# stm233/image-compression-for-machine

Measured on AMD Instinct MI355X. Metric: images/sec (256x256) cnn-hyperprior (WACNN) training step, higher is better.
Workload: dtype f32; 1 GPU; cnn (WACNN N=192 M=320) train step, lambda=0.0067 MSE, batch 16/GPU synthetic 256x256, Adam lr 1e-4 + aux Adam, clip 1.0; global_batch=16, parallelism=dp1

## Files before the change

### image-compression-for-machine_amd/csrc/conv_igemm.hip

```cpp
#include <cstdlib>
#include <vector>
#include "conv_common.h"

namespace icm {

template <int WCO, int WPX, int TCO, int TPX, int KS = 1>
__global__ __launch_bounds__(512, (TCO * TPX <= 3) ? 4 : 2) void conv_igemm_kernel(const ConvDesc d) {
  extern __shared__ __attribute__((aligned(16))) float smem[];
  static_assert(WCO * WPX * KS == 4, "4 MFMA waves per workgroup");
  constexpr int BCO_T = WCO * TCO;
  constexpr int TS = (TCO * TPX == 1) ? 3 : ((TCO * TPX == 2) ? 2 : 1);
  const int tid = threadIdx.x, lane = tid & 63, wave = tid >> 6;
  const bool loader = wave >= 4;
  const ConvPtrs P = d.g[blockIdx.y];
  const PatchGeom& pg = d.pg;

  int bid = xcd_block_id();
  const int cb = bid % d.ncb;
  int pt = bid / d.ncb;
  const int tx_i = pt % d.tiles_x;
  pt /= d.tiles_x;
  const int ty_i = pt % d.tiles_y;
  const int tn_i = pt / d.tiles_y;
  const int ox0 = tx_i << d.lgTW, oy0 = ty_i << d.lgTH, n0 = tn_i << d.lgTI;
  const int S_in = pg.S == 2 ? 2 : 1;
  const int iyb = oy0 * S_in + d.iy0, ixb = ox0 * S_in + d.ix0;
  const int bufsz = d.ckm * 8 * pg.CS;
  const int nchunks = (d.nchunks8 + d.ckm - 1) / d.ckm;

  if (loader) {
    const int lw = __builtin_amdgcn_readfirstlane(wave) - 4;
    PlaneMap pm;

    if (pg.dma) {
      plane_map_init(pm, pg, n0, iyb, ixb, lane);
      stage_planes_dma(P.x, pm, pg, 0, min(d.ckm, d.nchunks8) * 8, smem, lw, lane);
      asm volatile("s_waitcnt vmcnt(0)" ::: "memory");
      __syncthreads();
      for (int chunk = 0; chunk < nchunks; ++chunk) {
        if (chunk + 1 < nchunks) {
          const int c8 = (chunk + 1) * d.ckm;
          stage_planes_dma(P.x, pm, pg, c8 * 8, min(d.ckm, d.nchunks8 - c8) * 8, smem + ((chunk + 1) & 1) * bufsz, lw, lane);
          asm volatile("s_waitcnt vmcnt(0)" ::: "memory");
        }
        __syncthreads();
      }
      return;
    }
    if (pg.vec4) {
      plane_map_init_v4(pm, pg, n0, iyb, ixb, lane);
      stage_planes_v4<8>(P.x, pm, pg, 0, min(d.ckm, d.nchunks8) * 8, smem, lw);
      __syncthreads();
      for (int chunk = 0; chunk < nchunks; ++chunk) {
        if (chunk + 1 < nchunks) {
          const int c8 = (chunk + 1) * d.ckm;
          stage_planes_v4<8>(P.x, pm, pg, c8 * 8, min(d.ckm, d.nchunks8 - c8) * 8, smem + ((chunk + 1) & 1) * bufsz,
                             lw);
        }
        __syncthreads();
      }
      return;
    }
    plane_map_init(pm, pg, n0, iyb, ixb, lane);
    stage_planes<12>(P.x, pm, pg, 0, min(d.ckm, d.nchunks8) * 8, smem, lw);
    __syncthreads();
    for (int chunk = 0; chunk < nchunks; ++chunk) {
      if (chunk + 1 < nchunks) {
        const int c8 = (chunk + 1) * d.ckm;
        stage_planes<12>(P.x, pm, pg, c8 * 8, min(d.ckm, d.nchunks8 - c8) * 8, smem + ((chunk + 1) & 1) * bufsz, lw);
      }
      __syncthreads();
    }
    return;
  }

  const int wave_u = __builtin_amdgcn_readfirstlane(wave);
  const int wk = wave_u % KS, wsp = wave_u / KS;
  const int wco = wsp / WPX, wpx = wsp % WPX;
  const int h = lane >> 5, l31 = lane & 31;
  const int TWm = (1 << d.lgTW) - 1, THm = (1 << d.lgTH) - 1;
  const int rowmul = S_in * pg.PWrow;
  int boff[TPX];
#pragma unroll
  for (int tp = 0; tp < TPX; ++tp) {
    const int p = (wpx * TPX + tp) * 32 + l31;
    const int tx = p & TWm, ty = (p >> d.lgTW) & THm, ti = p >> (d.lgTW + d.lgTH);
    boff[tp] = h * pg.CS + ti * pg.PP + ty * rowmul + tx;
  }
  f32x16 acc[TCO][TPX];
#pragma unroll
  for (int a = 0; a < TCO; ++a)
#pragma unroll
    for (int b = 0; b < TPX; ++b)
#pragma unroll
      for (int r = 0; r < 16; ++r) acc[a][b][r] = 0.0f;

  const char* wbase = reinterpret_cast<const char*>(P.wp);
  const int cot0 = cb * BCO_T + wco * TCO;
  unsigned wl[TCO];
#pragma unroll
  for (int a = 0; a < TCO; ++a) wl[a] = (unsigned)(min(cot0 + a, d.ncot - 1) * 64 + lane) * 16u;
  const long long qstride = (long long)d.ncot * 64 * 16;
  const int Qtot = d.nchunks8 * d.ntaps;
  {
    int step_lane;
    {
      const int sq = lane / d.ntaps, tq = lane - sq * d.ntaps;
      step_lane = sq * 8 * pg.CS + d.tapoff[tq];
    }
    auto chunk_nq = [&](int c) { return min(d.ckm, d.nchunks8 - c * d.ckm) * d.ntaps; };
    auto steps2 = [&](int nq_c) { return ((((nq_c - wk + KS - 1) / KS) + TS - 1) / TS + 1) & ~1; };
    auto wptr = [&](int c, int st, int u) -> const char* {
      int nq_c = chunk_nq(c);
      const int ns2 = steps2(nq_c);
      if (st >= ns2) {
        st -= ns2;
        c += 1;
        nq_c = (c < nchunks) ? chunk_nq(c) : 1;
      }
      const int qw = min(c * d.ckm * d.ntaps + min((st * TS + u) * KS + wk, nq_c - 1), Qtot - 1);
      return wbase + qw * qstride;
    };
    f32x4 aq0[TS][TCO], aq1[TS][TCO];
#pragma unroll
    for (int u = 0; u < TS; ++u)
#pragma unroll
      for (int a = 0; a < TCO; ++a) {
        aq0[u][a] = *reinterpret_cast<const f32x4*>(wptr(0, 0, u) + wl[a]);
        aq1[u][a] = *reinterpret_cast<const f32x4*>(wptr(0, 1, u) + wl[a]);
      }

    __syncthreads();
    for (int chunk = 0; chunk < nchunks; ++chunk) {
      const float* cur = smem + (chunk & 1) * bufsz;
      const int nq = chunk_nq(chunk);
      const int nsteps2 = steps2(nq);
      float bv_n[TS][4][TPX];
      float ok_n[TS];
      auto bload = [&](int st, int u) {
        const int qq = (st * TS + u) * KS + wk;
        const int qc = min(qq, nq - 1);
        ok_n[u] = (qq < nq) ? 1.0f : 0.0f;
        const float* bp = cur + __builtin_amdgcn_readlane(step_lane, qc);
#pragma unroll
        for (int j = 0; j < 4; ++j)
#pragma unroll
          for (int tp = 0; tp < TPX; ++tp) bv_n[u][j][tp] = bp[boff[tp] + 2 * j * pg.CS];
      };
      auto half_step = [&](f32x4 (&aq)[TS][TCO], int st) {
        float bv[TS][4][TPX];
#pragma unroll
        for (int u = 0; u < TS; ++u)
#pragma unroll
          for (int j = 0; j < 4; ++j)
#pragma unroll
            for (int tp = 0; tp < TPX; ++tp) bv[u][j][tp] = bv_n[u][j][tp] * ok_n[u];
        const int stn = min(st + 1, nsteps2 - 1);
#pragma unroll
        for (int u = 0; u < TS; ++u) {
          const char* sp = wptr(chunk, st + 2, u);
#pragma unroll
          for (int a = 0; a < TCO; ++a) {
#pragma unroll
            for (int tp = 0; tp < TPX; ++tp)
#pragma unroll
              for (int j = 0; j < 4; ++j)
                acc[a][tp] = __builtin_amdgcn_mfma_f32_32x32x2f32(aq[u][a][j], bv[u][j][tp], acc[a][tp], 0, 0, 0);
            if (a == 0) bload(stn, u);
            aq[u][a] = *reinterpret_cast<const f32x4*>(sp + wl[a]);
            __builtin_amdgcn_sched_barrier(0);
          }
        }
      };
#pragma unroll
      for (int u = 0; u < TS; ++u) bload(0, u);
      for (int st = 0; st < nsteps2; st += 2) {
        half_step(aq0, st);
        half_step(aq1, st + 1);
      }
      __syncthreads();
    }
  }

  if constexpr (KS > 1) {
    static_assert(TCO == 1 && TPX == 1, "split-K configurations hold one tile per wave");
    float* red = smem + (wsp * (KS - 1)) * 1024;
    if (wk > 0) {
#pragma unroll
      for (int r = 0; r < 16; ++r) red[(wk - 1) * 1024 + r * 64 + lane] = acc[0][0][r];
    }
    __syncthreads();
    if (wk > 0) return;
#pragma unroll
    for (int k = 0; k < KS - 1; ++k)
#pragma unroll
      for (int r = 0; r < 16; ++r) acc[0][0][r] += red[k * 1024 + r * 64 + lane];
  }
  {
    int pn[TPX], poy[TPX], pox[TPX];
    bool pv[TPX];
#pragma unroll
    for (int tp = 0; tp < TPX; ++tp) {
      const int p = (wpx * TPX + tp) * 32 + l31;
      const int tx = p & TWm, ty = (p >> d.lgTW) & THm, ti = p >> (d.lgTW + d.lgTH);
      const int oyv = oy0 + ty, oxv = ox0 + tx;
      pn[tp] = n0 + ti;
      pv[tp] = (pn[tp] < d.pg.N) && (oyv < d.OHv) && (oxv < d.OWv);
      poy[tp] = oyv * d.out_sy + d.out_oy;
      pox[tp] = oxv * d.out_sx + d.out_ox;
    }
    epilogue_dispatch<TCO, TPX>(d, P, acc, cot0, h, pn, poy, pox, pv);
  }
}

struct PackDesc {
  const float* w;
  float* wp;
  int Co, Ci, KHW, src_out_major, ntaps, ncot, nchunks, nonneg;
  float bound, pedestal;
  int src_ld, src_off;
  int dst_ncot, dst_cot_off;
  int wino;
  short tapidx[ICM_MAX_TAPS];
};

#define ICM_PACK_LDS (8 * 32 * ICM_MAX_TAPS + 64)
__device__ __forceinline__ void pack_unit(const PackDesc& d, int cot, int chunk, float* lds) {
  const int KHW = d.KHW, tid = threadIdx.x;
  const int co0 = cot * 32, ci0 = chunk * 8;
  int rows, rlen, rstride;
  if (d.src_out_major) { rows = 32; rlen = 8 * KHW; } else { rows = 8; rlen = 32 * KHW; }
  rstride = rlen | 1;
  const int total = rows * rlen;
  for (int e0 = tid; e0 < total; e0 += 8 * (int)blockDim.x) {
    float v[8];
    int lo[8];
#pragma unroll
    for (int u = 0; u < 8; ++u) {
      const int e = e0 + u * (int)blockDim.x;
      v[u] = 0.0f;
      lo[u] = -1;
      if (e < total) {
        const int r = e / rlen, c = e - r * rlen;
        lo[u] = r * rstride + c;
        if (d.src_out_major) {
          const int co = co0 + r, ci = ci0 + c / KHW;
          if (co < d.Co && ci < d.Ci) v[u] = d.w[((long long)co * d.src_ld + d.src_off + ci0) * KHW + c];
        } else {
          const int ci = ci0 + r, co = co0 + c / KHW;
          if (ci < d.Ci && co < d.Co) v[u] = d.w[((long long)ci * d.src_ld + d.src_off + co0) * KHW + c];
        }
      }
    }
#pragma unroll
    for (int u = 0; u < 8; ++u) {
      if (lo[u] >= 0) {
        float x = v[u];
        if (d.nonneg) {
          x = fmaxf(x, d.bound);
          x = x * x - d.pedestal;
        }
        lds[lo[u]] = x;
      }
    }
  }
  __syncthreads();
  f32x4* out = reinterpret_cast<f32x4*>(d.wp);
  for (int e = tid; e < d.ntaps * 64; e += blockDim.x) {
    const int t = e >> 6, lane = e & 63;
    const int col = lane & 31, hh = lane >> 5, k = d.tapidx[t];
    f32x4 o;
#pragma unroll
    for (int j = 0; j < 4; ++j) {
      const int cil = 2 * j + hh;
      const float* gsrc = d.src_out_major ? lds + col * rstride + cil * KHW : lds + cil * rstride + col * KHW;
      float v;
      if (d.wino) {
        const int wa = t >> 2, wb = t & 3;
        float row[3];
#pragma unroll
        for (int p = 0; p < 3; ++p) {
          const float g0 = gsrc[d.wino == 2 ? (2 - p) * 3 + 2 : p * 3 + 0];
          const float g1 = gsrc[d.wino == 2 ? (2 - p) * 3 + 1 : p * 3 + 1];
          const float g2 = gsrc[d.wino == 2 ? (2 - p) * 3 + 0 : p * 3 + 2];
          row[p] = wb == 0 ? g0 : (wb == 3 ? g2 : (wb == 1 ? 0.5f * ((g0 + g2) + g1) : 0.5f * ((g0 + g2) - g1)));
        }
        v = wa == 0 ? row[0] : (wa == 3 ? row[2] : (wa == 1 ? 0.5f * ((row[0] + row[2]) + row[1]) : 0.5f * ((row[0] + row[2]) - row[1])));
      } else {
        v = gsrc[k];
      }
      const bool valid = (co0 + col < d.Co) && (ci0 + cil < d.Ci);
      o[j] = valid ? v : 0.0f;
    }
    out[((long long)(chunk * d.ntaps + t) * d.dst_ncot + d.dst_cot_off + cot) * 64 + lane] = o;
  }
  __syncthreads();
}

__global__ __launch_bounds__(256) void pack_weights_kernel(const PackDesc d) {
  __shared__ float lds[ICM_PACK_LDS];
  const int units = d.ncot * d.nchunks;
  for (int u = blockIdx.x; u < units; u += gridDim.x) pack_unit(d, u % d.ncot, u / d.ncot, lds);
}

#define ICM_PACK_NB 24
struct PackMulti {
  PackDesc g[ICM_PACK_NB];
};
__global__ __launch_bounds__(256) void pack_weights_multi_kernel(const PackMulti m) {
  __shared__ float lds[ICM_PACK_LDS];
  const PackDesc& d = m.g[blockIdx.y];
  const int units = d.ncot * d.nchunks;
  for (int u = blockIdx.x; u < units; u += gridDim.x) pack_unit(d, u % d.ncot, u / d.ncot, lds);
}

struct Tap {
  int kidx;
  int dy, dx;
};
struct ConvClass {
  int cy, cx;
  int iy0, ix0;
  int ey, ex;
  std::vector<Tap> taps;
};

static void axis_taps(int K, int s, int pad, int c, std::vector<int>& ks, std::vector<int>& dis) {
  for (int k = 0; k < K; ++k) {
    const int v = c + pad - k;
    if (((v % s) + s) % s != 0) continue;
    ks.push_back(k);
    dis.push_back(v >= 0 ? v / s : -((-v) / s));
  }
}

static std::vector<ConvClass> build_classes(int KH, int KW, int stride, int pad, int transposed) {
  std::vector<ConvClass> out;
  if (!transposed) {
    ConvClass c;
    c.cy = c.cx = 0;
    c.iy0 = c.ix0 = -pad;
    c.ey = KH;
    c.ex = KW;
    for (int kh = 0; kh < KH; ++kh)
      for (int kw = 0; kw < KW; ++kw) c.taps.push_back({kh * KW + kw, kh, kw});
    out.push_back(c);
    return out;
  }
  for (int cy = 0; cy < stride; ++cy)
    for (int cx = 0; cx < stride; ++cx) {
      std::vector<int> khs, dys, kws, dxs;
      axis_taps(KH, stride, pad, cy, khs, dys);
      axis_taps(KW, stride, pad, cx, kws, dxs);
      ConvClass c;
      c.cy = cy;
      c.cx = cx;
      int miny = 0, minx = 0, maxy = 0, maxx = 0;
      for (size_t i = 0; i < dys.size(); ++i) {
        miny = i ? std::min(miny, dys[i]) : dys[i];
        maxy = i ? std::max(maxy, dys[i]) : dys[i];
      }
      for (size_t i = 0; i < dxs.size(); ++i) {
        minx = i ? std::min(minx, dxs[i]) : dxs[i];
        maxx = i ? std::max(maxx, dxs[i]) : dxs[i];
      }
      c.iy0 = miny;
      c.ix0 = minx;
      c.ey = maxy - miny + 1;
      c.ex = maxx - minx + 1;
      for (size_t a = 0; a < khs.size(); ++a)
        for (size_t b = 0; b < kws.size(); ++b)
          c.taps.push_back({khs[a] * KW + kws[b], dys[a] - miny, dxs[b] - minx});
      out.push_back(c);
    }
  return out;
}

struct KernelCfg {
  int wco, wpx, tco, tpx;
  void (*fn)(const ConvDesc);
  int ks;
  double eff;
  int occ;
};
static const KernelCfg kCfgs[] = {
    {1, 4, 3, 2, conv_igemm_kernel<1, 4, 3, 2>, 1, 0.75, 1},
    {1, 4, 6, 1, conv_igemm_kernel<1, 4, 6, 1>, 1, 1.00, 1},
    {1, 4, 2, 2, conv_igemm_kernel<1, 4, 2, 2>, 1, 0.80, 1},
    {1, 4, 1, 2, conv_igemm_kernel<1, 4, 1, 2>, 1, 0.60, 2},
    {1, 4, 3, 1, conv_igemm_kernel<1, 4, 3, 1>, 1, 1.10, 2},
    {1, 4, 5, 1, conv_igemm_kernel<1, 4, 5, 1>, 1, 0.65, 1},
    {2, 2, 2, 1, conv_igemm_kernel<2, 2, 2, 1>, 1, 0.80, 2},
    {2, 2, 1, 1, conv_igemm_kernel<2, 2, 1, 1>, 1, 0.80, 2},
    {4, 1, 1, 1, conv_igemm_kernel<4, 1, 1, 1>, 1, 0.75, 2},
    {1, 4, 1, 1, conv_igemm_kernel<1, 4, 1, 1>, 1, 0.70, 2},
    {2, 1, 1, 1, conv_igemm_kernel<2, 1, 1, 1, 2>, 2, 0.70, 2},
    {1, 2, 1, 1, conv_igemm_kernel<1, 2, 1, 1, 2>, 2, 0.70, 2},
    {1, 1, 1, 1, conv_igemm_kernel<1, 1, 1, 1, 4>, 4, 0.65, 2},
};
constexpr int kNumCfgs = (int)(sizeof(kCfgs) / sizeof(kCfgs[0]));
static_assert(kNumCfgs <= ICM_CONV_CFG_KS8_64X64, "the K-split ids lie above the table rows");

static int g_force_cfg = ICM_CONV_CFG_AUTO;
static bool cfg_forced() { return g_force_cfg != ICM_CONV_CFG_AUTO; }
static bool ks8_forced() { return g_force_cfg == ICM_CONV_CFG_KS8_64X64 || g_force_cfg == ICM_CONV_CFG_KS8_32X128; }
static bool row_forced() { return cfg_forced() && g_force_cfg < ICM_CONV_CFG_KS8_64X64; }
static int g_force_1x1 = env_int("ICM_CONV_1X1", -1);

static Geometry make_geometry(int bpx, int OHv, int OWv, int N, int S, int ey, int ex, int nchunks8, int ntaps,
                              int tiles_per_wave) {
  Geometry g;
  const int lgB = ceil_log2(bpx);
  g.lgTW = std::min(std::min(5, lgB), ceil_log2(OWv));
  g.lgTH = std::min(lgB - g.lgTW, ceil_log2(OHv));
  g.lgTI = lgB - g.lgTW - g.lgTH;
  const int TW = 1 << g.lgTW, TH = 1 << g.lgTH, TI = 1 << g.lgTI;
  g.PW = (TW - 1) * S + ex;
  g.PH = (TH - 1) * S + ey;
  g.PWh = (g.PW + 1) / 2;
  g.PWrow = (S == 2) ? 2 * g.PWh : g.PW;
  g.PP = g.PH * g.PWrow;
  g.CS = TI * g.PP;
  g.tiles_x = cdiv(OWv, TW);
  g.tiles_y = cdiv(OHv, TH);
  g.tiles_n = cdiv(N, TI);
  int ckm = cdiv(256, ntaps * 4 * tiles_per_wave);
  ckm = std::max(1, std::min(ckm, nchunks8));
  ckm = std::max(1, std::min(ckm, 64 / std::max(1, ntaps)));
  while (ckm > 1 && (size_t)2 * ckm * 8 * g.CS * sizeof(float) > 64 * 1024) --ckm;
  g.ckm = ckm;
  g.lds_bytes = (size_t)2 * ckm * 8 * g.CS * sizeof(float);
  return g;
}
static bool fits_plane_map(const Geometry& g) { return (1 << g.lgTI) * g.PH * g.PW <= ICM_MAXJ * 64; }
static bool linear_patch(const Geometry& g) { return g.PWrow == g.PW && g.PP == g.PH * g.PW; }
static long long tile_count(const Geometry& g) { return (long long)g.tiles_x * g.tiles_y * g.tiles_n; }

struct ClassShape { int OHv, OWv, ncot, nchunks8, ntaps; };
static ClassShape class_shape(const icm_conv_args& a, const ConvClass& cls, int out_s) {
  return {a.transposed ? cdiv(a.OH - cls.cy, out_s) : a.OH, a.transposed ? cdiv(a.OW - cls.cx, out_s) : a.OW,
          cdiv(a.Cout, 32), cdiv(a.Cin, 8), (int)cls.taps.size()};
}

static int search_staged(const icm_conv_args& a, int ngroups, const ConvClass& cls, const ClassShape& s, int S_in,
                         Geometry& bg) {
  static const double kCoResBoost = env_double("ICM_CONV_BOOST", 1.25);
  int best = -1, best1 = -1;
  double best_cost = 1e300, best1_cost = 1e300;
  Geometry bg1{};
  for (int i = 0; i < kNumCfgs; ++i) {
    if (row_forced() && i != g_force_cfg) continue;
    const KernelCfg& c = kCfgs[i];
    const int bpx = c.wpx * c.tpx * 32, bco_t = c.wco * c.tco;
    Geometry g = make_geometry(bpx, s.OHv, s.OWv, a.N, S_in, cls.ey, cls.ex, s.nchunks8, s.ntaps, c.tco * c.tpx);
    if (c.ks > 1) g.lds_bytes = std::max<size_t>(g.lds_bytes, (size_t)(c.ks - 1) * c.wco * c.wpx * 4096);
    if (g.lds_bytes > 160 * 1024 || !fits_plane_map(g)) continue;
    const long long blocks = cdiv(s.ncot, bco_t) * tile_count(g) * ngroups;
    const int occ_max = (g.lds_bytes * 2 <= 160 * 1024) ? c.occ : 1;
    const int occ = (int)std::min<long long>(occ_max, (blocks + 255) / 256);
    const double rounds = (double)((blocks + 256 * occ - 1) / (256 * occ));
    const double mfma = (double)c.tco * c.tpx * s.nchunks8 * s.ntaps * 4 / c.ks + (c.ks > 1 ? 24.0 : 0.0);
    const double boost = occ > 1 ? 1.0 + (kCoResBoost - 1.0) * std::min(1.0, 1500.0 / mfma) : 1.0;
    const double cost = rounds * (occ * mfma / (c.eff * boost) + 200.0);
    if (s.ntaps >= 9 && (long long)s.OHv * s.OWv * a.N >= 16384 && cdiv(s.ncot, bco_t) == 1 && cost < best1_cost) {
      best1_cost = cost;
      best1 = i;
      bg1 = g;
    }
    if (cost < best_cost) {
      best_cost = cost;
      best = i;
      bg = g;
    }
  }
  if (best1 >= 0 && best1_cost <= 1.2 * best_cost) {
    best = best1;
    bg = bg1;
  }
  return best;
}

static int plan_ks8(const icm_conv_args& a, int ngroups, const ConvClass& cls, const ClassShape& s, int S_in, Geometry& g) {
  static const int ks8_on = env_int("ICM_CONV_KS8", 1);
  static const long long ks8_max = env_ll("ICM_CONV_KS8_MAXWG", 256);
  static const long long ks8_min = env_ll("ICM_CONV_KS8_MINWG", 160);
  if (!(ks8_forced() || (ks8_on && !cfg_forced())) || S_in != 1 || s.ntaps <= 1 || a.pro_act != ICM_ACT_NONE ||
      !EpiKs8::has(a.epi) || a.x_seg_len != 0)
    return 0;
  const int tco = g_force_cfg == ICM_CONV_CFG_KS8_32X128 ? 1 : (g_force_cfg == ICM_CONV_CFG_KS8_64X64 ? 2 : (s.ncot >= 2 ? 2 : 1));
  g = make_geometry(tco == 2 ? 64 : 128, s.OHv, s.OWv, a.N, S_in, cls.ey, cls.ex, s.nchunks8, s.ntaps, 4);
  int ckm = std::max(1, std::min(s.nchunks8, 64 / s.ntaps));
  while (ckm > 1 && (size_t)2 * ckm * 8 * g.CS * sizeof(float) > 96 * 1024) --ckm;
  g.ckm = ckm;
  g.lds_bytes = std::max((size_t)2 * ckm * 8 * g.CS * sizeof(float), (size_t)8 * 4 * 16 * 64 * sizeof(float));
  const long long blocks = cdiv(s.ncot, tco) * tile_count(g) * ngroups;
  const bool fits = g.lds_bytes <= 160 * 1024 && fits_plane_map(g) && linear_patch(g);
  return (fits && (ks8_forced() || (blocks <= ks8_max && blocks >= ks8_min && tco == 2))) ? tco : 0;
}

static int plan_class(const icm_conv_args& a, int ngroups, const ConvClass& cls, int S_in, int out_s, bool x_aligned16,
                      ConvPlan& p) {
  p = ConvPlan{};
  const ClassShape s = class_shape(a, cls, out_s);
  if (s.OHv <= 0 || s.OWv <= 0) return ICM_OK;
  if (s.ntaps > ICM_MAX_TAPS) return ICM_ERR_UNSUPPORTED;
  if (s.ntaps == 1 && S_in == 1 && out_s == 1 && cls.iy0 == 0 && cls.ix0 == 0 && a.x_seg_len == 0 && !cfg_forced()) {
    const int rc = plan_conv1x1(a, ngroups, g_force_1x1, p);
    if (rc >= 0) return rc;
  }
  p.row = search_staged(a, ngroups, cls, s, S_in, p.g);
  if (p.row < 0) return ICM_ERR_UNSUPPORTED;
  p.block = 512;
  Geometry kg;
  if (const int tco = plan_ks8(a, ngroups, cls, s, S_in, kg)) {
    p.family = kFamKs8;
    p.row = tco;
    p.g = kg;
    p.dma = 1;
  } else {
    const Geometry& g = p.g;
    const int plane4 = (1 << g.lgTI) * g.PH * (g.PW / 4);
    p.vec4 = S_in == 1 && cls.ex == 1 && cls.ey == 1 && cls.ix0 == 0 && (g.PW % 4) == 0 && ((1 << g.lgTW) % 4) == 0 &&
             (a.W % 4) == 0 && (a.x_bs % 4) == 0 && ((long long)a.H * a.W % 4) == 0 && plane4 <= 4 * 64 &&
             (g.CS % 4) == 0 && (g.PWrow % 4) == 0 && (g.PP % 4) == 0 && x_aligned16 && a.x_seg_len == 0;
    static const int dma_on = env_int("ICM_CONV_DMA", 1);
    p.dma = dma_on && !p.vec4 && S_in == 1 && a.pro_act == ICM_ACT_NONE && linear_patch(g);
  }
  p.ncb = cdiv(s.ncot, p.family == kFamKs8 ? p.row : kCfgs[p.row].wco * kCfgs[p.row].tco);
  p.nblk = p.ncb * tile_count(p.g);
  if (p.nblk <= 0 || p.nblk > 0x7fffffffLL) return ICM_ERR_ARG;
  return ICM_OK;
}

static int launch_class(const icm_conv_args* arr, int ngroups, const ConvClass& cls, long long wp_off, int S_in,
                        int out_s, const ConvPlan& p, hipStream_t stream) {
  if (p.nblk == 0) return ICM_OK;
  const icm_conv_args& a = arr[0];
  ConvDesc d{};
  fill_conv_desc(d, arr, ngroups, wp_off);
  d.ncb = p.ncb;
  if (p.family == kFam1x1) return launch_conv1x1(d, a, p, ngroups, stream);
  const ClassShape s = class_shape(a, cls, out_s);
  const Geometry& bg = p.g;
  PatchGeom& pg = d.pg;
  pg.PW = bg.PW; pg.PH = bg.PH; pg.PWrow = bg.PWrow; pg.PWh = bg.PWh; pg.PP = bg.PP; pg.CS = bg.CS; pg.S = S_in;
  pg.TIPH = (1 << bg.lgTI) * bg.PH;
  pg.dPW = make_fastdiv((uint32_t)bg.PW);
  pg.dTIPH = make_fastdiv((uint32_t)pg.TIPH);
  pg.dPH = make_fastdiv((uint32_t)bg.PH);
  pg.H = a.H; pg.W = a.W; pg.N = a.N; pg.C = a.Cin; pg.act = a.pro_act; pg.bs = a.x_bs;
  pg.seg_len = a.x_seg_len; pg.seg_gap = a.x_seg_len ? a.x_seg_gap : 0;
  pg.dseg = make_fastdiv((uint32_t)std::max(1, a.x_seg_len));
  pg.vec4 = p.vec4; pg.dma = p.dma; pg.pipe = 0;
  set_v4_pack(pg);
  d.ps2 = a.pixel_shuffle == 2;
  d.OHf = d.ps2 ? a.OH * 2 : a.OH;
  d.OWf = d.ps2 ? a.OW * 2 : a.OW;
  d.OHv = s.OHv; d.OWv = s.OWv;
  d.out_sy = d.out_sx = out_s;
  d.out_oy = cls.cy; d.out_ox = cls.cx;
  d.iy0 = cls.iy0; d.ix0 = cls.ix0;
  d.ntaps = s.ntaps;
  d.lgTW = bg.lgTW; d.lgTH = bg.lgTH; d.lgTI = bg.lgTI;
  d.tiles_x = bg.tiles_x; d.tiles_y = bg.tiles_y; d.tiles_n = bg.tiles_n;
  d.nchunks8 = s.nchunks8; d.ckm = bg.ckm;
  for (int t = 0; t < s.ntaps; ++t) {
    const Tap& tp = cls.taps[t];
    const int col = (S_in == 2) ? ((tp.dx & 1) * bg.PWh + (tp.dx >> 1)) : tp.dx;
    d.tapoff[t] = tp.dy * bg.PWrow + col;
  }
  if (p.family == kFamKs8) return launch_conv_ks8(d, p.row, p.nblk, ngroups, bg.lds_bytes, stream);
  const KernelCfg& c = kCfgs[p.row];
  if (bg.lds_bytes > 64 * 1024 && !ensure_max_lds(reinterpret_cast<const void*>(c.fn))) return ICM_ERR_LAUNCH;
  hipLaunchKernelGGL(c.fn, dim3((unsigned)p.nblk, ngroups, 1), dim3(p.block), bg.lds_bytes, stream, d);
  ICM_CHECK_LAUNCH();
  return ICM_OK;
}

static int validate(const icm_conv_args& a) {
  if (!a.x || !a.wp || !a.y) return ICM_ERR_ARG;
  if (a.N <= 0 || a.Cin <= 0 || a.Cout <= 0 || a.H <= 0 || a.W <= 0 || a.OH <= 0 || a.OW <= 0) return ICM_ERR_ARG;
  if (a.KH <= 0 || a.KW <= 0 || a.KH * a.KW > ICM_MAX_TAPS) return ICM_ERR_UNSUPPORTED;
  if (a.stride != 1 && a.stride != 2) return ICM_ERR_UNSUPPORTED;
  if (!a.transposed) {
    if (a.OH != (a.H + 2 * a.pad - a.KH) / a.stride + 1 || a.OW != (a.W + 2 * a.pad - a.KW) / a.stride + 1)
      return ICM_ERR_ARG;
  }
  if ((epi_reads_res(a.epi) && !a.res) || (epi_reads_aux(a.epi) && !a.aux) || (epi_reads_aux2(a.epi) && !a.aux2))
    return ICM_ERR_ARG;
  if (((long long)a.N * a.x_bs + 8LL * a.H * a.W) * 4 >= (1LL << 31)) return ICM_ERR_UNSUPPORTED;
  if (a.pixel_shuffle != 0 && a.pixel_shuffle != 2) return ICM_ERR_UNSUPPORTED;
  if (a.pixel_shuffle == 2 && (a.Cout % 4 != 0 || a.transposed)) return ICM_ERR_ARG;
  if (a.x_seg_len < 0 || (a.x_seg_len > 0 && (a.x_seg_gap < 0 || a.x_seg_len >= 65536))) return ICM_ERR_ARG;
  return ICM_OK;
}

static int check_group(const icm_conv_args* arr, int ngroups) {
  if (!arr || ngroups < 1 || ngroups > ICM_MAX_GROUPS) return ICM_ERR_ARG;
  for (int i = 0; i < ngroups; ++i) {
    int rc = validate(arr[i]);
    if (rc) return rc;
  }
  const icm_conv_args& a = arr[0];
  for (int i = 1; i < ngroups; ++i) {
    const icm_conv_args& b = arr[i];
    if (b.N != a.N || b.Cin != a.Cin || b.H != a.H || b.W != a.W || b.Cout != a.Cout || b.OH != a.OH || b.OW != a.OW ||
        b.KH != a.KH || b.KW != a.KW || b.stride != a.stride || b.pad != a.pad || b.transposed != a.transposed ||
        b.pro_act != a.pro_act || b.epi != a.epi || b.accum != a.accum || b.pixel_shuffle != a.pixel_shuffle ||
        b.x_bs != a.x_bs || b.y_bs != a.y_bs || b.x_seg_len != a.x_seg_len || b.x_seg_gap != a.x_seg_gap || b.algo != a.algo ||
        (b.res && b.res_bs != a.res_bs) || (b.aux && b.aux_bs != a.aux_bs) || (b.aux2 && b.aux2_bs != a.aux2_bs) ||
        (b.y2 && b.y2_bs != a.y2_bs) || (b.res != nullptr) != (a.res != nullptr) || (b.aux != nullptr) != (a.aux != nullptr) ||
        (b.aux2 != nullptr) != (a.aux2 != nullptr) || (b.y2 != nullptr) != (a.y2 != nullptr) ||
        (b.bias != nullptr) != (a.bias != nullptr) || (b.xv != nullptr) != (a.xv != nullptr))
      return ICM_ERR_ARG;
  }
  return (a.algo == ICM_ALGO_WINOGRAD || a.algo == ICM_ALGO_DIRECT) ? ICM_OK : ICM_ERR_ARG;
}

static long long class_packed_floats(int Cin, int ntaps, int ncot) { return (long long)cdiv(Cin, 8) * ntaps * ncot * 256; }

static bool x_aligned16(const icm_conv_args* arr, int ngroups) {
  bool ok = true;
  for (int gi = 0; gi < ngroups; ++gi) ok = ok && (reinterpret_cast<uintptr_t>(arr[gi].x) & 15) == 0;
  return ok;
}

static int conv_run_grouped(const icm_conv_args* arr, int ngroups, hipStream_t stream) {
  if (int rc = check_group(arr, ngroups)) return rc;
  const icm_conv_args& a = arr[0];
  if (a.algo == ICM_ALGO_WINOGRAD) return run_conv_wino(arr, ngroups, stream);
  const int S_in = a.transposed ? 1 : a.stride, out_s = a.transposed ? a.stride : 1;
  long long off = 0;
  for (const ConvClass& cls : build_classes(a.KH, a.KW, a.stride, a.pad, a.transposed)) {
    ConvPlan p;
    int rc = plan_class(a, ngroups, cls, S_in, out_s, x_aligned16(arr, ngroups), p);
    if (!rc) rc = launch_class(arr, ngroups, cls, off, S_in, out_s, p, stream);
    if (rc) return rc;
    off += class_packed_floats(a.Cin, (int)cls.taps.size(), cdiv(a.Cout, 32));
  }
  return ICM_OK;
}

static PackDesc make_pack_desc(const icm_pack_job& J, const ConvClass& cls, long long off) {
  const int ntaps = (int)cls.taps.size(), ncot = cdiv(J.Cout, 32);
  PackDesc d{};
  d.w = J.w;
  d.wp = J.wp + off;
  d.Co = J.Cout; d.Ci = J.Cin; d.KHW = J.KH * J.KW; d.src_out_major = J.src_out_major;
  d.ntaps = ntaps; d.ncot = ncot; d.nchunks = cdiv(J.Cin, 8); d.nonneg = J.nonneg;
  d.bound = J.bound; d.pedestal = J.pedestal;
  d.src_ld = J.src_ld > 0 ? J.src_ld : (J.src_out_major ? J.Cin : J.Cout); d.src_off = J.src_off;
  d.dst_ncot = J.dst_ncot > 0 ? J.dst_ncot : ncot; d.dst_cot_off = J.dst_cot_off; d.wino = J.wino;
  for (int t = 0; t < ntaps; ++t) d.tapidx[t] = (short)cls.taps[t].kidx;
  return d;
}

}

extern "C" {

int icm_conv_run(const icm_conv_args* a, void* stream) {
  return icm::conv_run_grouped(a, 1, (hipStream_t)stream);
}
int icm_conv_run_grouped(const icm_conv_args* a, int ngroups, void* stream) {
  return icm::conv_run_grouped(a, ngroups, (hipStream_t)stream);
}
int icm_conv2d_fwd(const icm_conv_args* a, void* stream) {
  if (!a || a->transposed) return ICM_ERR_ARG;
  return icm_conv_run(a, stream);
}
int icm_convT2d_dgrad(const icm_conv_args* a, void* stream) {
  if (!a || a->transposed) return ICM_ERR_ARG;
  return icm_conv_run(a, stream);
}
int icm_conv2d_dgrad(const icm_conv_args* a, void* stream) {
  if (!a || !a->transposed) return ICM_ERR_ARG;
  return icm_conv_run(a, stream);
}
int icm_convT2d_fwd(const icm_conv_args* a, void* stream) {
  if (!a || !a->transposed) return ICM_ERR_ARG;
  return icm_conv_run(a, stream);
}

int icm_conv_winograd_ok(const icm_conv_args* a) { return (a && icm::wino_supported(*a)) ? 1 : 0; }
int64_t icm_wino_transform_floats(const icm_conv_args* a) {
  return (a && icm::wino_supported(*a) && a->N > 0 && a->Cin > 0) ? (int64_t)icm::wino_transform_floats(*a) : -1;
}
int icm_wino_transform(const icm_conv_args* arr, int ngroups, void* stream) {
  if (!arr || ngroups < 1 || ngroups > ICM_MAX_GROUPS) return ICM_ERR_ARG;
  for (int i = 1; i < ngroups; ++i)
    if (arr[i].N != arr[0].N || arr[i].Cin != arr[0].Cin || arr[i].H != arr[0].H || arr[i].W != arr[0].W ||
        arr[i].x_bs != arr[0].x_bs || arr[i].pro_act != arr[0].pro_act || arr[i].x_seg_len != arr[0].x_seg_len ||
        arr[i].x_seg_gap != arr[0].x_seg_gap)
      return ICM_ERR_ARG;
  return icm::run_wino_transform(arr, ngroups, (hipStream_t)stream);
}

void icm_debug_force_conv_cfg(int idx) { icm::g_force_cfg = idx < 0 ? ICM_CONV_CFG_AUTO : idx; }
int icm_debug_forced_conv_cfg(void) { return icm::g_force_cfg; }
void icm_debug_force_conv1x1(int mode) { icm::g_force_1x1 = mode; }

int icm_debug_conv_plan(const icm_conv_args* arr, int ngroups, int cls, int64_t out[16]) {
  using namespace icm;
  std::fill(out, out + 16, 0);
  int rc = check_group(arr, ngroups);
  if (rc) return rc;
  const icm_conv_args& a = arr[0];
  if (a.algo == ICM_ALGO_WINOGRAD) {
    WinoPlan w{};
    if (cls != 0) return ICM_ERR_ARG;
    if ((rc = plan_conv_wino(a, ngroups, w))) return rc;
    const int64_t v[13] = {1, w.w8 ? kFamWino8 : kFamWino44, w.tco, w.g.lgTX, w.g.lgTY, w.g.lgTI, w.g.nsteps, w.ncb, w.nblk,
                           (int64_t)w.lds_bytes, 512, a.xv != nullptr, w.px_fast};
    std::copy(v, v + 13, out);
    return ICM_OK;
  }
  const std::vector<ConvClass> classes = build_classes(a.KH, a.KW, a.stride, a.pad, a.transposed);
  if (cls < 0 || cls >= (int)classes.size()) return ICM_ERR_ARG;
  long long off = 0;
  for (int i = 0; i < cls; ++i) off += class_packed_floats(a.Cin, (int)classes[i].taps.size(), cdiv(a.Cout, 32));
  ConvPlan p;
  rc = plan_class(a, ngroups, classes[cls], a.transposed ? 1 : a.stride, a.transposed ? a.stride : 1, x_aligned16(arr, ngroups), p);
  if (rc) return rc;
  const int64_t v[14] = {(int64_t)classes.size(), p.family, p.row, p.g.lgTW, p.g.lgTH, p.g.lgTI, p.g.ckm, p.ncb, p.nblk,
                         (int64_t)p.g.lds_bytes, p.block, p.vec4, p.dma, off};
  std::copy(v, v + 14, out);
  return ICM_OK;
}

int64_t icm_packed_weight_floats(int Cout, int Cin, int KH, int KW) {
  return icm::class_packed_floats(Cin, KH * KW, icm::cdiv(Cout, 32));
}

int icm_pack_weights(const float* w, float* wp, int Cout, int Cin, int KH, int KW, int src_out_major,
                     int transposed, int stride, int pad, int nonneg, float bound, float pedestal, void* stream) {
  using namespace icm;
  if (!w || !wp || Cout <= 0 || Cin <= 0 || KH * KW > ICM_MAX_TAPS || (stride != 1 && stride != 2)) return ICM_ERR_ARG;
  icm_pack_job J{};
  J.w = w; J.wp = wp; J.Cout = Cout; J.Cin = Cin; J.KH = KH; J.KW = KW; J.src_out_major = src_out_major; J.nonneg = nonneg;
  J.bound = bound; J.pedestal = pedestal;
  long long off = 0;
  for (const ConvClass& cls : build_classes(KH, KW, stride, pad, transposed)) {
    if (cls.taps.empty()) continue;
    const PackDesc d = make_pack_desc(J, cls, off);
    hipLaunchKernelGGL(pack_weights_kernel, dim3(std::min(d.nchunks * d.ncot, 2048)), dim3(256), 0, (hipStream_t)stream, d);
    ICM_CHECK_LAUNCH();
    off += class_packed_floats(Cin, d.ntaps, d.dst_ncot);
  }
  return ICM_OK;
}

int icm_pack_weights_batch(const icm_pack_job* jobs, int n, void* stream) {
  using namespace icm;
  if (!jobs || n < 1) return ICM_ERR_ARG;
  PackMulti m{};
  int nb = 0;
  auto flush = [&]() -> int {
    if (nb == 0) return ICM_OK;
    for (int i = nb; i < ICM_PACK_NB; ++i) m.g[i] = m.g[0];
    hipLaunchKernelGGL(pack_weights_multi_kernel, dim3(128, nb), dim3(256), 0, (hipStream_t)stream, m);
    ICM_CHECK_LAUNCH();
    nb = 0;
    return ICM_OK;
  };
  for (int k = 0; k < n; ++k) {
    const icm_pack_job& J = jobs[k];
    if (!J.w || !J.wp || J.Cout <= 0 || J.Cin <= 0 || J.KH * J.KW > ICM_MAX_TAPS || (J.stride != 1 && J.stride != 2))
      return ICM_ERR_ARG;
    std::vector<ConvClass> classes = build_classes(J.KH, J.KW, J.stride, J.pad, J.transposed);
    if (J.wino) {
      if (J.wino < 0 || J.wino > 2 || J.KH != 3 || J.KW != 3 || J.stride != 1 || J.pad != 1 || J.nonneg) return ICM_ERR_ARG;
      ConvClass wc;
      wc.cy = wc.cx = wc.iy0 = wc.ix0 = 0;
      wc.ey = wc.ex = 1;
      for (int t = 0; t < 16; ++t) wc.taps.push_back({0, 0, 0});
      classes.assign(1, wc);
    }
    const int ncot = cdiv(J.Cout, 32), inner = J.src_out_major ? J.Cin : J.Cout;
    if (J.src_off < 0 || J.src_off + inner > (J.src_ld > 0 ? J.src_ld : inner) || J.dst_cot_off < 0 ||
        J.dst_cot_off + ncot > (J.dst_ncot > 0 ? J.dst_ncot : ncot))
      return ICM_ERR_ARG;
    long long off = 0;
    for (const ConvClass& cls : classes) {
      if (cls.taps.empty()) continue;
      const PackDesc& d = m.g[nb] = make_pack_desc(J, cls, off);
      off += class_packed_floats(J.Cin, d.ntaps, d.dst_ncot);
      if (++nb == ICM_PACK_NB) {
        int rc = flush();
        if (rc) return rc;
      }
    }
  }
  return flush();
}

}
```

Baseline: 387.8 images/s.

## Rewrite weight-pack kernel with vectorized loads, multi-chunk runs and software pipelining

Restructures the weight packing kernel so each block processes runs of several input-channel chunks, loads source weights with 16-byte vector loads when aligned, and prefetches the next run into registers while emitting the current one. Jobs are flattened into a single 1D grid sized to resident capacity instead of a fixed 128xN grid, and Winograd transforms are computed once per row rather than per output tap. The goal is to cut the overhead and poor memory efficiency of per-step weight repacking. It adds complexity, register pressure from the 1D prefetch buffer, and a linear job lookup per run.

```diff
diff --git a/image-compression-for-machine_amd/csrc/conv_igemm.hip b/image-compression-for-machine_amd/csrc/conv_igemm.hip
--- a/image-compression-for-machine_amd/csrc/conv_igemm.hip
+++ b/image-compression-for-machine_amd/csrc/conv_igemm.hip
@@ -216,102 +216,220 @@
 struct PackDesc {
   const float* w;
   float* wp;
-  int Co, Ci, KHW, src_out_major, ntaps, ncot, nchunks, nonneg;
+  int Co, Ci, KHW, ntaps, ncot, nchunks;
   float bound, pedestal;
   int src_ld, src_off;
   int dst_ncot, dst_cot_off;
-  int wino;
-  short tapidx[ICM_MAX_TAPS];
+  int rchunks, nruns;
+  unsigned char src_out_major, nonneg;
+  unsigned char wino;
+  unsigned char vec4;
+  unsigned tapidx[ICM_MAX_TAPS / 4];
 };
 
 #define ICM_PACK_LDS (8 * 32 * ICM_MAX_TAPS + 64)
-__device__ __forceinline__ void pack_unit(const PackDesc& d, int cot, int chunk, float* lds) {
-  const int KHW = d.KHW, tid = threadIdx.x;
-  const int co0 = cot * 32, ci0 = chunk * 8;
-  int rows, rlen, rstride;
-  if (d.src_out_major) { rows = 32; rlen = 8 * KHW; } else { rows = 8; rlen = 32 * KHW; }
-  rstride = rlen | 1;
-  const int total = rows * rlen;
-  for (int e0 = tid; e0 < total; e0 += 8 * (int)blockDim.x) {
-    float v[8];
-    int lo[8];
-#pragma unroll
-    for (int u = 0; u < 8; ++u) {
-      const int e = e0 + u * (int)blockDim.x;
-      v[u] = 0.0f;
-      lo[u] = -1;
-      if (e < total) {
-        const int r = e / rlen, c = e - r * rlen;
-        lo[u] = r * rstride + c;
-        if (d.src_out_major) {
-          const int co = co0 + r, ci = ci0 + c / KHW;
-          if (co < d.Co && ci < d.Ci) v[u] = d.w[((long long)co * d.src_ld + d.src_off + ci0) * KHW + c];
+#define ICM_PACK_REGS ICM_MAX_TAPS
+struct PackRun {
+  int cot, chunk0, co0, ci0, nch;
+  int rows, seglen, rstride;
+  int nrows, vlen;
+  int pitch;
+  const float* src;
+};
+__device__ __forceinline__ PackRun pack_run(const PackDesc& d, int run) {
+  PackRun r;
+  const int g = run / d.ncot;
+  r.cot = run - g * d.ncot;
+  r.chunk0 = g * d.rchunks;
+  r.co0 = r.cot * 32;
+  r.ci0 = r.chunk0 * 8;
+  r.nch = min(d.rchunks, d.nchunks - r.chunk0);
+  const int nco = min(32, d.Co - r.co0), nci = min(r.nch * 8, d.Ci - r.ci0);
+  if (d.src_out_major) {
+    r.rows = 32; r.seglen = r.nch * 8 * d.KHW; r.nrows = nco; r.vlen = nci * d.KHW;
+    r.src = d.w + ((long long)r.co0 * d.src_ld + d.src_off + r.ci0) * d.KHW;
+  } else {
+    r.rows = r.nch * 8; r.seglen = 32 * d.KHW; r.nrows = nci; r.vlen = nco * d.KHW;
+    r.src = d.w + ((long long)r.ci0 * d.src_ld + d.src_off + r.co0) * d.KHW;
+  }
+  r.rstride = r.seglen | 1;
+  r.pitch = d.src_ld * d.KHW;
+  return r;
+}
+
+struct PackPos {
+  int row, c, srow, sc;
+  __device__ __forceinline__ PackPos(const PackRun& r, int W) {
+    const int e = (int)threadIdx.x * W, step = 256 * W;
+    row = e / r.seglen; c = e - row * r.seglen;
+    srow = step / r.seglen; sc = step - srow * r.seglen;
+  }
+  __device__ __forceinline__ void next(const PackRun& r) {
+    row += srow; c += sc;
+    if (c >= r.seglen) { c -= r.seglen; ++row; }
+  }
+};
+
+template <bool VEC>
+__device__ __forceinline__ void pack_load(const PackRun& r, float (&v)[ICM_PACK_REGS]) {
+  constexpr int W = VEC ? 4 : 1, NV = ICM_PACK_REGS / W;
+  const int total = r.rows * r.seglen;
+  PackPos p(r, W);
+#pragma unroll
+  for (int u0 = 0; u0 < NV; u0 += 4) {
+    if (u0 * 256 * W < total) {
+#pragma unroll
+      for (int u = u0; u < u0 + 4; ++u) {
+        const bool ok = p.row < r.nrows && p.c < r.vlen;
+        const float* a = r.src + (ok ? p.row * r.pitch + p.c : 0);
+        if constexpr (VEC) {
+          const f32x4 q = *reinterpret_cast<const f32x4*>(a);
+#pragma unroll
+          for (int k = 0; k < 4; ++k) v[u * 4 + k] = q[k];
         } else {
-          const int ci = ci0 + r, co = co0 + c / KHW;
-          if (ci < d.Ci && co < d.Co) v[u] = d.w[((long long)ci * d.src_ld + d.src_off + co0) * KHW + c];
+          v[u] = *a;
         }
-      }
-    }
-#pragma unroll
-    for (int u = 0; u < 8; ++u) {
-      if (lo[u] >= 0) {
-        float x = v[u];
-        if (d.nonneg) {
-          x = fmaxf(x, d.bound);
-          x = x * x - d.pedestal;
+        p.next(r);
+      }
+    }
+  }
+}
+
+template <bool VEC>
+__device__ __forceinline__ void pack_stage(const PackDesc& d, const PackRun& r, const float (&v)[ICM_PACK_REGS], float* lds) {
+  constexpr int W = VEC ? 4 : 1, NV = ICM_PACK_REGS / W;
+  const int total = r.rows * r.seglen;
+  PackPos p(r, W);
+#pragma unroll
+  for (int u0 = 0; u0 < NV; u0 += 4) {
+    if (u0 * 256 * W < total) {
+#pragma unroll
+      for (int u = u0; u < u0 + 4; ++u) {
+        if (p.row < r.rows) {
+          const bool ok = p.row < r.nrows && p.c < r.vlen;
+#pragma unroll
+          for (int k = 0; k < W; ++k) {
+            float x = ok ? v[u * W + k] : 0.0f;
+            if (d.nonneg) {
+              x = fmaxf(x, d.bound);
+              x = __builtin_fmaf(x, x, -d.pedestal);
+            }
+            lds[p.row * r.rstride + p.c + k] = x;
+          }
         }
-        lds[lo[u]] = x;
-      }
-    }
-  }
-  __syncthreads();
-  f32x4* out = reinterpret_cast<f32x4*>(d.wp);
-  for (int e = tid; e < d.ntaps * 64; e += blockDim.x) {
-    const int t = e >> 6, lane = e & 63;
-    const int col = lane & 31, hh = lane >> 5, k = d.tapidx[t];
-    f32x4 o;
-#pragma unroll
-    for (int j = 0; j < 4; ++j) {
-      const int cil = 2 * j + hh;
-      const float* gsrc = d.src_out_major ? lds + col * rstride + cil * KHW : lds + cil * rstride + col * KHW;
-      float v;
-      if (d.wino) {
-        const int wa = t >> 2, wb = t & 3;
-        float row[3];
+        p.next(r);
+      }
+    }
+  }
+}
+
+__device__ __forceinline__ void pack_emit(const PackDesc& d, const PackRun& r, const float* lds) {
+  const int lane = threadIdx.x & 63, col = lane & 31, hh = lane >> 5;
+  const int wv = __builtin_amdgcn_readfirstlane((int)threadIdx.x >> 6);
+  const int cs = d.src_out_major ? r.rstride : d.KHW, is = d.src_out_major ? d.KHW : r.rstride;
+  const bool cov = r.co0 + col < d.Co;
+  const float* src = lds + col * cs + hh * is;
+  f32x4* out = reinterpret_cast<f32x4*>(d.wp) + (long long)(d.dst_cot_off + r.cot) * 64 + lane;
+  const long long tstride = (long long)d.dst_ncot * 64;
+  if (d.wino) {
+    const int g00 = d.wino == 2 ? 8 : 0, gs = d.wino == 2 ? -1 : 1;
+    for (int cl = wv; cl < r.nch; cl += 4) {
+      float gg[4][3][4];
+      bool valid[4];
+#pragma unroll
+      for (int j = 0; j < 4; ++j) {
+        const float* g = src + (cl * 8 + 2 * j) * is + g00;
+        valid[j] = cov && (r.ci0 + cl * 8 + 2 * j + hh < d.Ci);
 #pragma unroll
         for (int p = 0; p < 3; ++p) {
-          const float g0 = gsrc[d.wino == 2 ? (2 - p) * 3 + 2 : p * 3 + 0];
-          const float g1 = gsrc[d.wino == 2 ? (2 - p) * 3 + 1 : p * 3 + 1];
-          const float g2 = gsrc[d.wino == 2 ? (2 - p) * 3 + 0 : p * 3 + 2];
-          row[p] = wb == 0 ? g0 : (wb == 3 ? g2 : (wb == 1 ? 0.5f * ((g0 + g2) + g1) : 0.5f * ((g0 + g2) - g1)));
+          const float g0 = g[gs * (p * 3 + 0)], g1 = g[gs * (p * 3 + 1)], g2 = g[gs * (p * 3 + 2)];
+          gg[j][p][0] = g0;
+          gg[j][p][1] = 0.5f * ((g0 + g2) + g1);
+          gg[j][p][2] = 0.5f * ((g0 + g2) - g1);
+          gg[j][p][3] = g2;
         }
-        v = wa == 0 ? row[0] : (wa == 3 ? row[2] : (wa == 1 ? 0.5f * ((row[0] + row[2]) + row[1]) : 0.5f * ((row[0] + row[2]) - row[1])));
-      } else {
-        v = gsrc[k];
-      }
-      const bool valid = (co0 + col < d.Co) && (ci0 + cil < d.Ci);
-      o[j] = valid ? v : 0.0f;
-    }
-    out[((long long)(chunk * d.ntaps + t) * d.dst_ncot + d.dst_cot_off + cot) * 64 + lane] = o;
-  }
-  __syncthreads();
-}
-
-__global__ __launch_bounds__(256) void pack_weights_kernel(const PackDesc d) {
-  __shared__ float lds[ICM_PACK_LDS];
-  const int units = d.ncot * d.nchunks;
-  for (int u = blockIdx.x; u < units; u += gridDim.x) pack_unit(d, u % d.ncot, u / d.ncot, lds);
+      }
+      f32x4* o16 = out + (long long)(r.chunk0 + cl) * 16 * tstride;
+#pragma unroll
+      for (int a = 0; a < 4; ++a) {
+#pragma unroll
+        for (int b = 0; b < 4; ++b) {
+          f32x4 o;
+#pragma unroll
+          for (int j = 0; j < 4; ++j) {
+            const float r0 = gg[j][0][b], r1 = gg[j][1][b], r2 = gg[j][2][b];
+            const float u = a == 0 ? r0 : (a == 3 ? r2 : (a == 1 ? 0.5f * ((r0 + r2) + r1) : 0.5f * ((r0 + r2) - r1)));
+            o[j] = valid[j] ? u : 0.0f;
+          }
+          o16[(a * 4 + b) * tstride] = o;
+        }
+      }
+    }
+  } else {
+    const int items = r.nch * d.ntaps, scl = 4 / d.ntaps, st = 4 - scl * d.ntaps;
+    int cl = wv / d.ntaps, t = wv - cl * d.ntaps;
+    for (int q = wv; q < items; q += 4) {
+      const int k = (d.tapidx[t >> 2] >> (8 * (t & 3))) & 255;
+      f32x4 o;
+#pragma unroll
+      for (int j = 0; j < 4; ++j) {
+        const float x = src[(cl * 8 + 2 * j) * is + k];
+        const bool valid = cov && (r.ci0 + cl * 8 + 2 * j + hh < d.Ci);
+        o[j] = valid ? x : 0.0f;
+      }
+      out[((long long)(r.chunk0 + cl) * d.ntaps + t) * tstride] = o;
+      cl += scl; t += st;
+      if (t >= d.ntaps) { t -= d.ntaps; ++cl; }
+    }
+  }
 }
 
 #define ICM_PACK_NB 24
 struct PackMulti {
   PackDesc g[ICM_PACK_NB];
+  int first_run[ICM_PACK_NB + 1];
+  int njobs;
 };
+static_assert(sizeof(PackMulti) <= 4096, "kernel arguments are limited to 4 KB");
+
+__device__ __forceinline__ int pack_job_of(const PackMulti& m, int run) {
+  int j = 0;
+  while (j + 1 < m.njobs && run >= m.first_run[j + 1]) ++j;
+  return __builtin_amdgcn_readfirstlane(j);
+}
+__device__ __forceinline__ void pack_load_any(const PackDesc& d, const PackRun& r, float (&v)[ICM_PACK_REGS]) {
+  if (d.vec4) pack_load<true>(r, v);
+  else pack_load<false>(r, v);
+}
+
 __global__ __launch_bounds__(256) void pack_weights_multi_kernel(const PackMulti m) {
   __shared__ float lds[ICM_PACK_LDS];
-  const PackDesc& d = m.g[blockIdx.y];
-  const int units = d.ncot * d.nchunks;
-  for (int u = blockIdx.x; u < units; u += gridDim.x) pack_unit(d, u % d.ncot, u / d.ncot, lds);
+  const int total = m.first_run[m.njobs];
+  int run = blockIdx.x;
+  if (run >= total) return;
+  float v[ICM_PACK_REGS];
+  int job = pack_job_of(m, run);
+  PackRun r = pack_run(m.g[job], run - m.first_run[job]);
+  pack_load_any(m.g[job], r, v);
+  for (;;) {
+    const PackDesc& d = m.g[job];
+    if (d.vec4) pack_stage<true>(d, r, v, lds);
+    else pack_stage<false>(d, r, v, lds);
+    __syncthreads();
+    const int nrun = run + (int)gridDim.x;
+    const bool more = nrun < total;
+    int njob = job;
+    PackRun nr = r;
+    if (more) {
+      njob = pack_job_of(m, nrun);
+      nr = pack_run(m.g[njob], nrun - m.first_run[njob]);
+      pack_load_any(m.g[njob], nr, v);
+    }
+    pack_emit(d, r, lds);
+    if (!more) break;
+    __syncthreads();
+    run = nrun; job = njob; r = nr;
+  }
 }
 
 struct Tap {
@@ -646,13 +764,48 @@
   PackDesc d{};
   d.w = J.w;
   d.wp = J.wp + off;
-  d.Co = J.Cout; d.Ci = J.Cin; d.KHW = J.KH * J.KW; d.src_out_major = J.src_out_major;
-  d.ntaps = ntaps; d.ncot = ncot; d.nchunks = cdiv(J.Cin, 8); d.nonneg = J.nonneg;
+  d.Co = J.Cout; d.Ci = J.Cin; d.KHW = J.KH * J.KW; d.src_out_major = J.src_out_major != 0;
+  d.ntaps = ntaps; d.ncot = ncot; d.nchunks = cdiv(J.Cin, 8); d.nonneg = J.nonneg != 0;
   d.bound = J.bound; d.pedestal = J.pedestal;
   d.src_ld = J.src_ld > 0 ? J.src_ld : (J.src_out_major ? J.Cin : J.Cout); d.src_off = J.src_off;
-  d.dst_ncot = J.dst_ncot > 0 ? J.dst_ncot : ncot; d.dst_cot_off = J.dst_cot_off; d.wino = J.wino;
-  for (int t = 0; t < ntaps; ++t) d.tapidx[t] = (short)cls.taps[t].kidx;
+  d.dst_ncot = J.dst_ncot > 0 ? J.dst_ncot : ncot; d.dst_cot_off = J.dst_cot_off; d.wino = (unsigned char)J.wino;
+  for (int t = 0; t < ntaps; ++t) d.tapidx[t >> 2] |= (unsigned)cls.taps[t].kidx << (8 * (t & 3));
+  const int inner = J.src_out_major ? J.Cin : J.Cout;
+  d.vec4 = (reinterpret_cast<uintptr_t>(J.w) & 15) == 0 && ((long long)d.src_ld * d.KHW) % 4 == 0 &&
+           ((long long)d.src_off * d.KHW) % 4 == 0 && ((long long)inner * d.KHW) % 4 == 0;
+  auto lds_floats = [&](int r) { return d.src_out_major ? 32 * ((r * 8 * d.KHW) | 1) : r * 8 * ((32 * d.KHW) | 1); };
+  d.rchunks = std::max(1, std::min({ICM_MAX_TAPS / d.KHW, 16, d.nchunks}));
+  while (d.rchunks > 1 && lds_floats(d.rchunks) > ICM_PACK_LDS) --d.rchunks;
   return d;
+}
+
+static constexpr int kPackResident = 256 * 3;
+static int launch_pack(PackMulti& m, int nb, hipStream_t stream) {
+  auto count = [&]() {
+    int total = 0;
+    for (int i = 0; i < nb; ++i) {
+      PackDesc& d = m.g[i];
+      d.nruns = d.ncot * cdiv(d.nchunks, d.rchunks);
+      m.first_run[i] = total;
+      total += d.nruns;
+    }
+    for (int i = nb; i <= ICM_PACK_NB; ++i) m.first_run[i] = total;
+    return total;
+  };
+  int total = count();
+  for (bool shorter = true; total < kPackResident && shorter; total = count()) {
+    shorter = false;
+    for (int i = 0; i < nb; ++i)
+      if (m.g[i].rchunks > 1) {
+        m.g[i].rchunks = (m.g[i].rchunks + 1) / 2;
+        shorter = true;
+      }
+  }
+  m.njobs = nb;
+  const int grid = cdiv(total, cdiv(total, kPackResident));
+  hipLaunchKernelGGL(pack_weights_multi_kernel, dim3(grid), dim3(256), 0, stream, m);
+  ICM_CHECK_LAUNCH();
+  return ICM_OK;
 }
 
 }
@@ -734,20 +887,10 @@
 
 int icm_pack_weights(const float* w, float* wp, int Cout, int Cin, int KH, int KW, int src_out_major,
                      int transposed, int stride, int pad, int nonneg, float bound, float pedestal, void* stream) {
-  using namespace icm;
-  if (!w || !wp || Cout <= 0 || Cin <= 0 || KH * KW > ICM_MAX_TAPS || (stride != 1 && stride != 2)) return ICM_ERR_ARG;
   icm_pack_job J{};
-  J.w = w; J.wp = wp; J.Cout = Cout; J.Cin = Cin; J.KH = KH; J.KW = KW; J.src_out_major = src_out_major; J.nonneg = nonneg;
-  J.bound = bound; J.pedestal = pedestal;
-  long long off = 0;
-  for (const ConvClass& cls : build_classes(KH, KW, stride, pad, transposed)) {
-    if (cls.taps.empty()) continue;
-    const PackDesc d = make_pack_desc(J, cls, off);
-    hipLaunchKernelGGL(pack_weights_kernel, dim3(std::min(d.nchunks * d.ncot, 2048)), dim3(256), 0, (hipStream_t)stream, d);
-    ICM_CHECK_LAUNCH();
-    off += class_packed_floats(Cin, d.ntaps, d.dst_ncot);
-  }
-  return ICM_OK;
+  J.w = w; J.wp = wp; J.Cout = Cout; J.Cin = Cin; J.KH = KH; J.KW = KW; J.src_out_major = src_out_major;
+  J.transposed = transposed; J.stride = stride; J.pad = pad; J.nonneg = nonneg; J.bound = bound; J.pedestal = pedestal;
+  return icm_pack_weights_batch(&J, 1, stream);
 }
 
 int icm_pack_weights_batch(const icm_pack_job* jobs, int n, void* stream) {
@@ -757,11 +900,9 @@
   int nb = 0;
   auto flush = [&]() -> int {
     if (nb == 0) return ICM_OK;
-    for (int i = nb; i < ICM_PACK_NB; ++i) m.g[i] = m.g[0];
-    hipLaunchKernelGGL(pack_weights_multi_kernel, dim3(128, nb), dim3(256), 0, (hipStream_t)stream, m);
-    ICM_CHECK_LAUNCH();
+    const int rc = launch_pack(m, nb, (hipStream_t)stream);
     nb = 0;
-    return ICM_OK;
+    return rc;
   };
   for (int k = 0; k < n; ++k) {
     const icm_pack_job& J = jobs[k];
```

New measurement: 391.5 images/s, median of 6. No clear change (+1.0%).
